# karenyang/GCN-VAE

Measured on NVIDIA B200. Metric: train edges/s (fwd+bwd) + eval triples/s, FB15k-237 shape, 1/2/4/8 B200, higher is better.
Workload: dtype f32

## Files before the change

### gcn-vae_b200/_lib.py

```python
import ctypes
import os

import torch

HERE = os.path.dirname(os.path.abspath(__file__))
LIB_PATH = os.path.join(HERE, "libkgvae_b200.so")

_P, _I, _F, _L, _Z = ctypes.c_void_p, ctypes.c_int, ctypes.c_float, ctypes.c_longlong, ctypes.c_size_t

_SIGNATURES = {
    "kg_last_error": (ctypes.c_char_p, []),
    "kg_version": (_I, []),
    "kg_device_info": (_I, [_P, _P, _P]),
    "kg_peer_alloc": (_I, [_Z, _P, _P]),
    "kg_peer_open": (_I, [_P, _P]),
    "kg_peer_close": (_I, [_P]),
    "kg_peer_free": (_I, [_P]),
    "kg_graph_build_workspace_bytes": (_Z, [_I]),
    "kg_graph_build": (_I, [_P, _P, _P, _I, _I, _I, _P, _P, _P, _P, _P, _P, _P, _P, _P, _P, _P, _Z, _P]),
    "kg_graph_index_workspace_bytes": (_Z, [_I]),
    "kg_graph_index": (_I, [_P, _P, _P, _P, _I, _I, _I, _P, _P, _P, _P, _P, _P, _P, _Z, _P]),
    "kg_embedding_fwd": (_I, [_P, _P, _I, _I, _P, _P]),
    "kg_embedding_bwd": (_I, [_P, _P, _I, _I, _P, _P]),
    "kg_bdd_weight_layouts": (_I, [_P, _I, _I, _I, _I, _P, _P, _P]),
    "kg_bdd_rel_fwd": (_I, [_P, _P, _I, _P, _I, _P, _P, _I, _I, _I, _P, _I, _P]),
    "kg_bdd_rel_bwd": (_I, [_P, _P, _I, _P, _P, _I, _P, _P, _I, _I, _I, _P, _P, _I, _P]),
    "kg_bdd_rel_fwd_cols": (_I, [_P, _P, _I, _P, _I, _I, _I, _I, _I, _P, _I, _P]),
    "kg_bdd_rel_bwd_cols": (_I, [_P, _P, _P, _I, _P, _I, _I, _I, _I, _I, _P, _P, _I, _P]),
    "kg_bdd_layouts_needed": (_I, [_I, _I, _I]),
    "kg_graph_rel_tiled_workspace_bytes": (_Z, [_I]),
    "kg_graph_rel_tiled": (_I, [_P, _P, _P, _P, _I, _I, _I, _I, _I, _P, _P, _Z, _P]),
    "kg_basis_id_fwd": (_I, [_P, _P, _P, _P, _P, _I, _I, _I, _I, _P, _P]),
    "kg_basis_id_bwd": (_I, [_P, _P, _P, _P, _P, _I, _I, _I, _I, _P, _P, _P]),
    "kg_basis_id_src_eligible": (_I, [_I, _I, _I]),
    "kg_basis_id_src_fwd": (_I, [_P, _P, _P, _P, _I, _I, _I, _I, _P, _P]),
    "kg_basis_id_src_bwd": (_I, [_P, _P, _P, _P, _P, _I, _I, _I, _I, _P, _P, _P]),
    "kg_basis_dense_fwd": (_I, [_P, _P, _I, _P, _I, _I, _I, _P, _P]),
    "kg_basis_dense_bwd": (_I, [_P, _P, _P, _I, _P, _I, _I, _I, _P, _P, _P]),
    "kg_act_dropout_bwd": (_I, [_P, _P, _P, _I, _L, _P, _P]),
    "kg_act_dropout_bwd_colsum": (_I, [_P, _P, _P, _I, _I, _I, _P, _P, _P, _Z, _P]),
    "kg_colsum_workspace_bytes": (_Z, [_I, _I]),
    "kg_colsum": (_I, [_P, _I, _I, _P, _P, _Z, _P]),
    "kg_gemm_f32_workspace_bytes": (_Z, [_I, _I, _I]),
    "kg_gemm_f32": (_I, [_P, _I, _I, _P, _I, _I, _P, _I, _I, _I, _I, _P, _P, _I, _P, _I, _P, _Z, _P]),
    "kg_gemm_f32_uses_tensor_cores": (_I, [_I, _I, _I]),
    "kg_gemm_prep_bytes": (_Z, [_I, _I]),
    "kg_gemm_prepare": (_I, [_P, _I, _I, _I, _P, _Z, _P]),
    "kg_gemm_f32_prepared_workspace_bytes": (_Z, [_I, _I, _I]),
    "kg_gemm_f32_prepared": (_I, [_P, _I, _P, _I, _P, _I, _I, _I, _I, _P, _P, _I, _P, _I, _P, _Z, _P]),
    "kg_reparam_fwd": (_I, [_P, _P, _I, _I, _P, _P, _P, _P]),
    "kg_reparam_bwd": (_I, [_P, _P, _P, _P, _P, _P, _I, _I, _P, _P]),
    "kg_kl_mog_fwd": (_I, [_P, _P, _P, _P, _I, _I, _I, _P, _P, _P, _P]),
    "kg_kl_mog_bwd": (_I, [_P, _P, _P, _P, _P, _P, _F, _I, _I, _I, _P, _P, _P, _P, _P]),
    "kg_kl_mog_bwd_fused": (_I, [_P, _P, _P, _P, _P, _P, _F, _I, _I, _I, _P, _P, _P, _P, _P, _P, _P]),
    "kg_iaf_update_fwd": (_I, [_P, _P, _P, _P, _I, _I, _P, _P, _P]),
    "kg_iaf_update_bwd": (_I, [_P, _P, _P, _P, _P, _I, _I, _P, _P, _P, _P]),
    "kg_reverse_columns": (_I, [_P, _I, _I, _P, _P]),
    "kg_distmult_score": (_I, [_P, _P, _P, _I, _I, _P, _P, _P]),
    "kg_reduce_workspace_bytes": (_Z, [_L]),
    "kg_bce_logits_fwd": (_I, [_P, _P, _I, _P, _P, _P, _Z, _P]),
    "kg_sum_squares": (_I, [_P, _L, _P, _P, _Z, _P]),
    "kg_sum": (_I, [_P, _L, _P, _P, _Z, _P]),
    "kg_triplet_index_workspace_bytes": (_Z, [_I]),
    "kg_triplet_index": (_I, [_P, _I, _I, _I, _P, _P, _P, _P, _Z, _P]),
    "kg_distmult_bce_workspace_bytes": (_Z, [_I]),
    "kg_distmult_bce_fwd": (_I, [_P, _P, _P, _P, _I, _I, _P, _P, _P, _P, _P, _P, _P, _P, _Z, _P]),
    "kg_distmult_bwd_dz": (_I, [_P, _P, _P, _P, _P, _I, _I, _P, _P]),
    "kg_triplet_index_trailing": (_I, [_P, _I, _I, _I, _P, _P, _P, _P, _Z, _P]),
    "kg_distmult_bce_fwd_lead": (_I, [_P, _P, _P, _P, _I, _I, _P, _P, _P, _P, _P, _P, _P, _P, _Z, _P]),
    "kg_distmult_bwd_dz_trailing": (_I, [_P, _P, _P, _P, _P, _I, _I, _P, _P]),
    "kg_distmult_bwd_dw": (_I, [_P, _P, _P, _I, _I, _P, _P]),
    "kg_distmult_rank_workspace_bytes": (_Z, [_I, _I, _I]),
    "kg_distmult_rank": (_I, [_P, _P, _P, _P, _P, _I, _I, _I, _P, _I, _I, _P, _P, _P, _Z, _P, _P, _P]),
    "kg_probe_l2": (_I, [_P, _P, _I, _I, _L, _I, _P, _P]),
    "kg_set_tc_terms": (_I, [_I]),
    "kg_distmult_topk_workspace_bytes": (_Z, [_I, _I, _I, _I]),
    "kg_distmult_topk": (_I, [_P, _P, _P, _P, _I, _I, _I, _P, _I, _P, _Z, _P, _P, _P]),
}

_lib = None


def lib():
    global _lib
    if _lib is None:
        if not os.path.exists(LIB_PATH):
            raise RuntimeError(
                f"kgvae_b200: {LIB_PATH} is missing - build it with "
                "`python -c 'import __graft_entry__ as g; g.build()'` (there is no CPU fallback)")
        handle = ctypes.CDLL(LIB_PATH)
        for name, (res, args) in _SIGNATURES.items():
            fn = getattr(handle, name)
            fn.restype, fn.argtypes = res, args
        _lib = handle
    return _lib


KERNELS_PER_CALL = {
    "kg_graph_build": 14, "kg_graph_index": 10, "kg_graph_rel_tiled": 5, "kg_triplet_index": 13, "kg_triplet_index_trailing": 18, "kg_distmult_bce_fwd": 5, "kg_distmult_bce_fwd_lead": 5, "kg_colsum": 2, "kg_act_dropout_bwd_colsum": 1,
    "kg_gemm_f32": 5,
    "kg_gemm_prepare": 2,
    "kg_kl_mog_fwd": 2, "kg_bce_logits_fwd": 2, "kg_sum_squares": 2, "kg_sum": 2, "kg_distmult_rank": 3, "kg_distmult_topk": 5,
}
launches = 0
profile = None


_seen_dev = None


def call(name, *args, tag=None):
    global launches, _seen_dev
    handle = lib()
    if _seen_dev is not None:
        dev, _seen_dev = _seen_dev, None
        if dev != torch.cuda.current_device():
            raise RuntimeError(f"kgvae_b200: {name} was given tensors on cuda:{dev} while the current device is "
                               f"cuda:{torch.cuda.current_device()} (use torch.cuda.set_device / torch.cuda.device)")
    if profile is not None:
        ev0, ev1 = torch.cuda.Event(enable_timing=True), torch.cuda.Event(enable_timing=True)
        ev0.record()
    rc = getattr(handle, name)(*args)
    if rc != 0:
        raise RuntimeError(f"{name} failed ({rc}): {handle.kg_last_error().decode()}")
    launches += KERNELS_PER_CALL.get(name, 1)
    if profile is not None:
        ev1.record()
        profile.setdefault(tag or name, []).append((ev0, ev1))


def ptr(t, dtype=None):
    if t is None:
        return None
    if not t.is_cuda:
        raise RuntimeError("kgvae_b200 ops need CUDA tensors (no CPU fallback)")
# ... 34 lines not shown
```

### gcn-vae_b200/csrc/latent.cu

```cuda
#include "common.cuh"

static constexpr int kThreads = 256;
static constexpr int kMaxMix = 16;
#define KG_LOG_SQRT_2PI 0.91893853320467274178f

__global__ void reparam_fwd_kernel(const float* __restrict__ h2, const float* __restrict__ eps, int n,
                                   int h, float* __restrict__ zm, float* __restrict__ zv,
                                   float* __restrict__ z) {
  long long t = (long long)blockIdx.x * blockDim.x + threadIdx.x;
  if (t >= (long long)n * h) return;
  int i = (int)(t / h), d = (int)(t % h);
  const float m = h2[(size_t)i * 2 * h + d];
  const float v = kg_softplus(h2[(size_t)i * 2 * h + h + d]) + 1e-8f;
  zm[t] = m;
  zv[t] = v;
  z[t] = m + eps[t] * sqrtf(v);
}

__global__ void reparam_bwd_kernel(const float* __restrict__ h2, const float* __restrict__ eps,
                                   const float* __restrict__ zv, const float* __restrict__ dz,
                                   const float* __restrict__ dmean, const float* __restrict__ dvar,
                                   int n, int h, float* __restrict__ dh2) {
  long long t = (long long)blockIdx.x * blockDim.x + threadIdx.x;
  if (t >= (long long)n * h) return;
  int i = (int)(t / h), d = (int)(t % h);
  const float g = dz ? dz[t] : 0.f;
  float gm = g, gv = g * eps[t] * 0.5f / sqrtf(zv[t]);
  if (dmean) gm += dmean[t];
  if (dvar) gv += dvar[t];
  dh2[(size_t)i * 2 * h + d] = gm;
  dh2[(size_t)i * 2 * h + h + d] = gv * kg_sigmoid(h2[(size_t)i * 2 * h + h + d]);
}
// ... 210 lines not shown
static void launch_kl_bwd(dim3 grid, cudaStream_t st, const float* z, const float* zm, const float* zv, const float* z_pre,
                          const float* ws, const float* resp, float scale, int n, int h, int k, const float* coefs,
                          const float* add, float* dz, float* dmean, float* dvar, float* dz_pre) {
  if (k <= 4) kl_mog_bwd_kernel<4><<<grid, 128, 0, st>>>(z, zm, zv, z_pre, ws, resp, scale, n, h, k, coefs, add, dz, dmean, dvar, dz_pre);
  else if (k <= 8) kl_mog_bwd_kernel<8><<<grid, 128, 0, st>>>(z, zm, zv, z_pre, ws, resp, scale, n, h, k, coefs, add, dz, dmean, dvar, dz_pre);
  else if (k <= 12) kl_mog_bwd_kernel<12><<<grid, 128, 0, st>>>(z, zm, zv, z_pre, ws, resp, scale, n, h, k, coefs, add, dz, dmean, dvar, dz_pre);
  else kl_mog_bwd_kernel<16><<<grid, 128, 0, st>>>(z, zm, zv, z_pre, ws, resp, scale, n, h, k, coefs, add, dz, dmean, dvar, dz_pre);
}

extern "C" int kg_kl_mog_bwd(const float* z, const float* z_mean, const float* z_var,
                             const float* z_pre, const float* prior_ws, const float* resp, float scale,
                             int n, int h, int k, float* dz, float* dmean, float* dvar, float* dz_pre,
                             void* stream) {
  KG_REQUIRE(n >= 0 && h > 0 && k > 0 && k <= kMaxMix, "kl bwd: need 0 < k <= 16");
  if (n == 0) return KG_OK;
  dim3 grid(kg_div_up(n, kKlRows), kg_div_up(h, 128));
  launch_kl_bwd(grid, kg_stream(stream), z, z_mean, z_var, z_pre, prior_ws, resp, scale, n, h, k, nullptr, nullptr, dz,
                dmean, dvar, dz_pre);
  KG_LAUNCH_OK();
  return KG_OK;
}

extern "C" int kg_kl_mog_bwd_fused(const float* z, const float* z_mean, const float* z_var,
                                   const float* z_pre, const float* prior_ws, const float* resp, float scale,
                                   int n, int h, int k, const float* coefs, const float* add, float* dz,
                                   float* dmean, float* dvar, float* dz_pre, void* stream) {
  KG_REQUIRE(n >= 0 && h > 0 && k > 0 && k <= kMaxMix, "kl bwd: need 0 < k <= 16");
  KG_REQUIRE(coefs != nullptr, "kl bwd fused: coefs is required");
  if (n == 0) return KG_OK;
  dim3 grid(kg_div_up(n, kKlRows), kg_div_up(h, 128));
  launch_kl_bwd(grid, kg_stream(stream), z, z_mean, z_var, z_pre, prior_ws, resp, scale, n, h, k, coefs, add, dz, dmean,
                dvar, dz_pre);
  KG_LAUNCH_OK();
  return KG_OK;
}

__global__ void __launch_bounds__(kThreads)
iaf_update_fwd_kernel(const float* __restrict__ z, const float* __restrict__ net,
                      const float* __restrict__ x_old, const int* __restrict__ col_mult, int n, int d,
                      float* __restrict__ x_new, float* __restrict__ log_det) {
  const int row = (int)(((long long)blockIdx.x * blockDim.x + threadIdx.x) >> 5);
  const int lane = threadIdx.x & 31;
  if (row >= n) return;
  const float* mu = net + (size_t)row * 2 * d;
  const float* alpha = mu + d;
  float s = 0.f;
  for (int j = lane; j < d; j += 32) {
    const float al = alpha[j];
    s += al;
    const size_t off = (size_t)row * d + j;
    if (__ldg(col_mult + j) == 0) x_new[off] = x_old[off];
    else x_new[off] = z[off] * expf(al + mu[j]);
  }
  if (log_det) {
    s = kg_warp_sum(s);
    if (lane == 0) log_det[row] = s;
  }
}

__global__ void iaf_update_bwd_kernel(const float* __restrict__ z, const float* __restrict__ net,
                                      const float* __restrict__ dx_new,
                                      const float* __restrict__ dlog_det,
                                      const int* __restrict__ col_mult, int n, int d,
                                      float* __restrict__ dz, float* __restrict__ dnet,
                                      float* __restrict__ dx_old) {
  long long t = (long long)blockIdx.x * blockDim.x + threadIdx.x;
// ... 58 lines not shown
```

### gcn-vae_b200/link_predict.py

```python
import argparse
import time

import numpy as np
import torch
import torch.nn as nn

from . import datasets, ops, utils
from .model import KGVAE, RGCN


class LinkPredict(nn.Module):
    def __init__(self, model_class, in_dim, h_dim, num_rels, num_bases=-1, num_hidden_layers=1,
                 dropout=0, use_cuda=True, reg_param=0, kl_param=0, mmd_param=0, k=1, n_flows=0):
        super().__init__()
        kwargs = dict(num_nodes=in_dim, h_dim=h_dim, out_dim=h_dim, num_rels=num_rels * 2,
                      num_bases=num_bases, num_hidden_layers=num_hidden_layers, dropout=dropout,
                      use_self_loop=use_cuda, use_cuda=use_cuda)
        if model_class is KGVAE:
            kwargs.update(k=k, n_flows=n_flows)
        self.encoder = model_class(**kwargs)
        self.reg_param, self.kl_param, self.mmd_param = reg_param, kl_param, mmd_param
        self.w_relation = nn.Parameter(torch.Tensor(num_rels, h_dim))
        self.use_cuda, self.k, self.n_flows = use_cuda, k, n_flows
        nn.init.xavier_uniform_(self.w_relation, gain=nn.init.calculate_gain("relu"))

    def grad_buckets(self, group=None, average=True, sharded=()):
        from . import parallel
        skip = {id(p) for p in sharded}
        enc = self.encoder
        named = dict(self.named_parameters())
        pick = lambda prefix: [p for n, p in named.items() if n.startswith(prefix) and p.requires_grad and id(p) not in skip]
        head = [p for n, p in named.items() if p.requires_grad and id(p) not in skip and
                not n.startswith(("encoder.rconv_layer_", "encoder.input_layer", "encoder.layers"))]
        order = [head, pick("encoder.rconv_layer_2"), pick("encoder.rconv_layer_1"), pick("encoder.layers"),
                 pick("encoder.input_layer")]
        params = [p for p in self.parameters() if p.requires_grad and id(p) not in skip]
        return parallel.GradBuckets(params, buckets=[b for b in order if b], group=group, average=average)

    def release_graph(self):
        enc = self.encoder
        for name in ("z_mean", "z_sigma", "log_det_sum", "flow_log_prob"):
            v = getattr(enc, name, None)
            if isinstance(v, torch.Tensor) and v.grad_fn is not None:
                setattr(enc, name, v.detach())

    def _flow_shift(self):
        if self.n_flows > 0 and isinstance(self.encoder, KGVAE):
            return self.encoder.get_flow_log_prob()
        return None

    def calc_score(self, embedding, triplets, shift=None):
        trip = ops.as_i32(triplets, embedding.device)
        return ops.DistMultScoreFn.apply(embedding, self.w_relation, trip, shift)

    def forward(self, g, h, r, norm):
        return self.encoder.forward(g, h, r, norm)

    def regularization_loss(self, embedding):
        return ops.MeanSquareFn.apply(embedding) + ops.MeanSquareFn.apply(self.w_relation)

    def get_loss(self, g, embed, triplets, labels):
        if getattr(g, "partition", None) is not None:
            return self._get_loss_partitioned(g.partition, embed, triplets, labels)
        trip = ops.as_i32(triplets, embed.device)
        lab = torch.as_tensor(labels, dtype=torch.float32, device=embed.device)
        zero = lambda: torch.zeros(1, device=embed.device)
        enc = self.encoder
        if isinstance(enc, KGVAE) and embed.requires_grad:
            flp = enc.flow_log_prob if enc.n_flows > 0 else None
            head, predict_loss, reg_loss, kl_core = ops.LossHeadFn.apply(
                embed, enc.z_mean, enc.z_sigma, enc.z_pre, self.w_relation, trip, lab, self._flow_shift(),
                self.reg_param, self.kl_param)
            kl = (kl_core if flp is None else kl_core + flp) if self.kl_param > 0 else zero()
            mmd = enc.get_mmd(embed) if self.mmd_param > 0 else zero()
            loss = head
            if self.kl_param > 0 and flp is not None:
                loss = loss + self.kl_param * flp
            if self.mmd_param > 0:
                loss = loss + self.mmd_param * mmd
            return loss, predict_loss, kl, mmd
        predict_loss = ops.DistMultBceFn.apply(embed, self.w_relation, trip, lab, self._flow_shift())
        reg_loss = self.regularization_loss(embed)
        kl = self.encoder.get_kl(embed) if self.kl_param > 0 else zero()
        mmd = self.encoder.get_mmd(embed) if self.mmd_param > 0 else zero()
        loss = predict_loss + self.reg_param * reg_loss + self.kl_param * kl + self.mmd_param * mmd
        return loss, predict_loss, kl, mmd


    def _get_loss_partitioned(self, part, embed, triplets, labels):
        from . import parallel
        dev = embed.device
        trip = ops.as_i32(triplets, dev)
        lab = torch.as_tensor(labels, dtype=torch.float32, device=dev)
        counts = torch.tensor([float(trip.shape[0])], device=dev)
        torch.distributed.all_reduce(counts, group=part.group)
        pending_z = parallel.allgather_rows_start(embed.detach(), part)
        frac = part.n_local / part.n_global
        reg_loss = ops.MeanSquareFn.apply(embed) * frac + ops.MeanSquareFn.apply(self.w_relation) / part.world_size
        zero = lambda: torch.zeros(1, device=dev)
        if self.kl_param > 0:
# ... 286 lines not shown
```

### gcn-vae_b200/model.py

```python
import random

import numpy as np
import torch
import torch.nn as nn
import torch.nn.functional as F

from . import ops, utils
from .flow_network import MADE, PermuteLayer
from .nn import RelGraphConv


class EmbeddingLayer(nn.Module):

    def __init__(self, num_nodes, h_dim):
        super().__init__()
        self.embedding = nn.Embedding(num_nodes, h_dim)

    def forward(self, g, h, r, norm):
        ids = ops.as_i32(h.reshape(-1), self.embedding.weight.device)
        return ops.EmbeddingFn.apply(self.embedding.weight, ids)


class KGVAE(nn.Module):

    def __init__(self, num_nodes, h_dim, out_dim, num_rels, num_bases, num_hidden_layers=1,
                 dropout=0, use_self_loop=False, use_cuda=True, k=10, n_flows=0):
        super().__init__()
        self.num_nodes, self.h_dim, self.out_dim, self.num_rels = num_nodes, h_dim, out_dim, num_rels
        self.num_bases = None if num_bases < 0 else num_bases
        self.num_hidden_layers = num_hidden_layers
        self.dropout = dropout
        self.use_self_loop, self.use_cuda = use_self_loop, use_cuda
        self.k = k
        self.flow_log_prob = None
        self.preset_eps = None
        self.build_encoder()
        self.z_pre = nn.Parameter(torch.randn(1, 2 * k, h_dim) / np.sqrt(k * h_dim))
        self.pi = nn.Parameter(torch.ones(k) / k, requires_grad=False)
        self.n_flows = n_flows
        if n_flows > 0:
            self.build_iaf()

    def build_iaf(self):
        blocks = []
        for _ in range(self.n_flows):
            blocks += [MADE(self.h_dim, self.h_dim, self.n_flows), PermuteLayer(self.h_dim)]
        self.nf = nn.Sequential(*blocks)

    def build_encoder(self):
        self.input_layer = EmbeddingLayer(self.num_nodes, self.h_dim)
        self.rconv_layer_1 = RelGraphConv(self.h_dim, self.h_dim, self.num_rels, "bdd",
                                          self.num_bases, activation=nn.ReLU(), self_loop=True,
                                          dropout=self.dropout)
        self.rconv_layer_2 = RelGraphConv(self.h_dim, self.h_dim * 2, self.num_rels, "bdd",
                                          self.num_bases, activation=nn.Identity(), self_loop=True,
                                          dropout=self.dropout)

    def forward(self, g, h, r, norm):
        self.node_id = h.squeeze()
        x = self.input_layer(g, h, r, norm)
        x = self.rconv_layer_1(g, x, r, norm)
        x = self.rconv_layer_2(g, x, r, norm)
        eps = self.preset_eps
        if eps is None:
            part = getattr(g, "partition", None)
            gen = None if part is None else part.noise_generator(x.device)
            eps = torch.randn((x.shape[0], self.h_dim), device=x.device, generator=gen)
        self.z_mean, self.z_sigma, z = ops.ReparamFn.apply(x, eps)
        if self.n_flows > 0:
            log_det_sum = None
            for flow in self.nf:
                z, log_det = flow.forward(z)
                if isinstance(flow, MADE):
                    log_det_sum = log_det if log_det_sum is None else log_det_sum + log_det
            self.log_det_sum = log_det_sum
            part = getattr(g, "partition", None)
            if part is None:
                self.flow_log_prob = torch.mean(log_det_sum)
            else:
                from . import parallel
                self.flow_log_prob = parallel.AllReduceSumFn.apply(log_det_sum.sum(), part.group) / part.n_global
        return z

    def get_kl(self, z):
        kl = ops.KlMogFn.apply(z, self.z_mean, self.z_sigma, self.z_pre)
        return kl if self.flow_log_prob is None else kl + self.flow_log_prob

    def get_flow_log_prob(self):
        return self.flow_log_prob

    def compute_kernel(self, x, y):
        d = x.size(1)
        diff = x.unsqueeze(1) - y.unsqueeze(0)
        return torch.exp(-diff.pow(2).mean(2) / float(d))

    def get_mmd(self, z):
        m_mix, s_mix = utils.gaussian_parameters(self.z_pre, dim=1)
        num_sample = 200
        z_pri = utils.sample_gaussian(m_mix, s_mix, repeat=num_sample // self.k)
        if self.n_flows > 0:
# ... 91 lines not shown
```

### gcn-vae_b200/ops.py

```python
import os

import torch

from . import _lib as L


def _c(t):
    return t if t.is_contiguous() else t.contiguous()


class tensor_core_terms:

    def __init__(self, terms):
        self.terms = int(terms)

    def __enter__(self):
        self.old = L.lib().kg_set_tc_terms(self.terms)
        return self

    def __exit__(self, *exc):
        L.lib().kg_set_tc_terms(self.old)
        return False


# ... 353 lines not shown
        if ctx.has_bias and ctx.needs_input_grad[3]:
            dbias = dbias_fused
        if isinstance(pending, list):
            dx = torch.cat([p_.wait() for p_ in pending], dim=1) if pending else None
        elif pending is not None:
            dx = pending.wait()
        return dx, dw, dloop, dbias, None, None, None, None, None, None, None


class ReparamFn(torch.autograd.Function):

    @staticmethod
    def forward(ctx, h2, eps):
        h2, eps = _c(h2), _c(eps)
        n, h = eps.shape
        zm, zv, z = (torch.empty_like(eps) for _ in range(3))
        L.call("kg_reparam_fwd", L.f32(h2), L.f32(eps), n, h, L.f32(zm), L.f32(zv), L.f32(z), L.stream())
        ctx.save_for_backward(h2, eps, zv)
        return zm, zv, z

    @staticmethod
    def backward(ctx, gm, gv, gz):
        h2, eps, zv = ctx.saved_tensors
        n, h = eps.shape
        gm = None if gm is None else _c(gm)
        gv = None if gv is None else _c(gv)
        gz = None if gz is None else _c(gz)
        dh2 = torch.empty_like(h2)
        L.call("kg_reparam_bwd", L.f32(h2), L.f32(eps), L.f32(zv), L.f32(gz), L.f32(gm), L.f32(gv),
               n, h, L.f32(dh2), L.stream())
        return dh2, None


class KlMogFn(torch.autograd.Function):

    @staticmethod
    def forward(ctx, z, z_mean, z_var, z_pre):
        z, z_mean, z_var = _c(z), _c(z_mean), _c(z_var)
        zp = _c(z_pre.reshape(-1, z_pre.shape[-1]))
        n, h = z.shape
        k = zp.shape[0] // 2
        dev = z.device
        ws = torch.empty((3, k, h), dtype=torch.float32, device=dev)
        rows = torch.empty(n, dtype=torch.float32, device=dev)
        resp = torch.empty((n, k), dtype=torch.float32, device=dev)
        L.call("kg_kl_mog_fwd", L.f32(z), L.f32(z_mean), L.f32(z_var), L.f32(zp), n, h, k, L.f32(ws),
               L.f32(rows), L.f32(resp), L.stream())
        ctx.save_for_backward(z, z_mean, z_var, zp, ws, resp)
        ctx.pre_shape = z_pre.shape
        return _reduce("kg_sum", rows) / n

    @staticmethod
    def backward(ctx, g):
        z, z_mean, z_var, zp, ws, resp = ctx.saved_tensors
        n, h = z.shape
        k = zp.shape[0] // 2
        dz, dm, dv = (torch.empty_like(z) for _ in range(3))
        dzp = torch.zeros_like(zp)
        L.call("kg_kl_mog_bwd", L.f32(z), L.f32(z_mean), L.f32(z_var), L.f32(zp), L.f32(ws),
               L.f32(resp), 1.0 / n, n, h, k, L.f32(dz), L.f32(dm), L.f32(dv), L.f32(dzp), L.stream())
        return dz * g, dm * g, dv * g, (dzp * g).view(ctx.pre_shape)


class LinearFn(torch.autograd.Function):

    @staticmethod
# ... 228 lines not shown
        ctx.shift_shape = None if shift is None else shift.shape
        ctx.pre_shape = None if z_pre is None else z_pre.shape
        return loss, pred, reg, kl

    @staticmethod
    def backward(ctx, g_loss, g_pred, g_reg, g_kl):
        saved = ctx.saved_tensors
        z, w, dz_pred, dw, out = saved[:5]
        n, h = z.shape
        zero = torch.zeros((), dtype=torch.float32, device=z.device)
        g_loss, g_pred, g_reg, g_kl = ((zero if t is None else t.reshape(()).to(torch.float32))
                                       for t in (g_loss, g_pred, g_reg, g_kl))
        c_pred = g_loss + g_pred
        c_reg = g_loss * ctx.reg_param + g_reg
        c_kl = g_loss * ctx.kl_param + g_kl
        dm = dv = dzp = None
        if ctx.use_kl:
            z_mean, z_var, zp, pws, resp = saved[5:]
            k = zp.shape[0] // 2
            coefs = torch.stack([c_kl, c_pred, c_reg * (2.0 / z.numel())]).contiguous()
            dz, dm, dv = (torch.empty_like(z) for _ in range(3))
            dzp = torch.zeros_like(zp)
            L.call("kg_kl_mog_bwd_fused", L.f32(z), L.f32(z_mean), L.f32(z_var), L.f32(zp), L.f32(pws), L.f32(resp),
                   1.0 / n, n, h, k, L.f32(coefs), L.f32(dz_pred), L.f32(dz), L.f32(dm), L.f32(dv), L.f32(dzp),
                   L.stream(), tag="kg_kl_mog_bwd")
            dzp = dzp.view(ctx.pre_shape)
        else:
            dz = torch.addcmul(dz_pred * c_pred, z, c_reg * (2.0 / z.numel()))
        dwo = torch.addcmul(dw * c_pred, w, c_reg * (2.0 / w.numel()))
        dshift = (out[1] * c_pred).reshape(ctx.shift_shape) if ctx.shift_shape is not None else None
        return dz, dm, dv, dzp, dwo, None, None, dshift, None, None


class BceLogitsFn(torch.autograd.Function):

    @staticmethod
    def forward(ctx, score, labels):
        score, labels = _c(score), _c(labels)
        n = score.numel()
        loss = torch.empty((), dtype=torch.float32, device=score.device)
        dscore = torch.empty_like(score)
        ws = L.workspace(L.lib().kg_reduce_workspace_bytes(n), score.device)
        L.call("kg_bce_logits_fwd", L.f32(score), L.f32(labels), n, L.f32(loss), L.f32(dscore),
               L.ptr(ws), ws.numel(), L.stream())
        ctx.save_for_backward(dscore)
        return loss

    @staticmethod
    def backward(ctx, g):
        (dscore,) = ctx.saved_tensors
        return dscore * g, None


class MeanSquareFn(torch.autograd.Function):

    @staticmethod
    def forward(ctx, x):
        x = _c(x)
        ctx.save_for_backward(x)
        return _reduce("kg_sum_squares", x) / x.numel()

    @staticmethod
    def backward(ctx, g):
        (x,) = ctx.saved_tensors
        return x * (g * (2.0 / x.numel()))

# ... 27 lines not shown
```

### include/kgvae_b200.h

```cpp
#ifndef KGVAE_B200_H_
#define KGVAE_B200_H_

#include <stddef.h>
#include <stdint.h>

#ifdef __cplusplus
extern "C" {
#endif

#define KG_OK 0
#define KG_ERR_INVALID -1
#define KG_ERR_CUDA -2
#define KG_ERR_WORKSPACE -3

const char* kg_last_error(void);
int kg_version(void);
int kg_device_info(int* sm_count, int* cc_major, int* cc_minor);
int kg_peer_alloc(size_t bytes, void** ptr, unsigned char* handle_out );
int kg_peer_open(const unsigned char* handle , void** ptr);
int kg_peer_close(void* ptr);
int kg_peer_free(void* ptr);

size_t kg_graph_build_workspace_bytes(int n_triplets);
int kg_graph_build(const int32_t* src, const int32_t* rel, const int32_t* dst, int n_triplets,
// ... 68 lines not shown
int kg_colsum(const float* x, int rows, int cols, float* out, void* workspace, size_t workspace_bytes,
              void* stream);

size_t kg_gemm_f32_workspace_bytes(int M, int N, int K);
int kg_gemm_f32(const float* A, int lda, int trans_a, const float* B, int ldb, int trans_b,
                float* C, int ldc, int M, int N, int K,
                const float* bias, const float* addend, int relu, const float* mask,
                int accumulate, void* workspace, size_t workspace_bytes, void* stream);

int kg_gemm_f32_uses_tensor_cores(int M, int N, int K);
size_t kg_gemm_prep_bytes(int rows, int cols);
int kg_gemm_prepare(const float* src, int ld, int rows, int cols, void* prep, size_t prep_bytes, void* stream);
size_t kg_gemm_f32_prepared_workspace_bytes(int M, int N, int K);
int kg_gemm_f32_prepared(const void* prep_a, int trans_a, const void* prep_b, int trans_b,
                         float* C, int ldc, int M, int N, int K,
                         const float* bias, const float* addend, int relu, const float* mask,
                         int accumulate, void* workspace, size_t workspace_bytes, void* stream);

int kg_reparam_fwd(const float* h2, const float* eps, int n, int h, float* z_mean, float* z_var,
                   float* z, void* stream);
int kg_reparam_bwd(const float* h2, const float* eps, const float* z_var, const float* dz,
                   const float* dmean, const float* dvar, int n, int h, float* dh2, void* stream);

int kg_kl_mog_fwd(const float* z, const float* z_mean, const float* z_var, const float* z_pre,
                  int n, int h, int k, float* prior_ws, float* kl_rows, float* resp, void* stream);
int kg_kl_mog_bwd(const float* z, const float* z_mean, const float* z_var, const float* z_pre,
                  const float* prior_ws, const float* resp, float scale, int n, int h, int k,
                  float* dz, float* dmean, float* dvar, float* dz_pre, void* stream);
int kg_kl_mog_bwd_fused(const float* z, const float* z_mean, const float* z_var, const float* z_pre,
                        const float* prior_ws, const float* resp, float scale, int n, int h, int k,
                        const float* coefs, const float* add, float* dz, float* dmean, float* dvar,
                        float* dz_pre, void* stream);

int kg_iaf_update_fwd(const float* z, const float* net_out, const float* x_old,
                      const int32_t* col_mult, int n, int d, float* x_new, float* log_det,
                      void* stream);
int kg_iaf_update_bwd(const float* z, const float* net_out, const float* dx_new,
                      const float* dlog_det , const int32_t* col_mult, int n, int d,
                      float* dz, float* dnet_out, float* dx_old, void* stream);
int kg_reverse_columns(const float* x, int n, int d, float* out, void* stream);

int kg_distmult_score(const float* z, const float* w, const int32_t* triplets, int n_triplets, int h,
                      const float* shift , float* score, void* stream);
size_t kg_reduce_workspace_bytes(long long n);
int kg_bce_logits_fwd(const float* score, const float* labels, int n, float* loss_out, float* dscore,
                      void* workspace, size_t workspace_bytes, void* stream);
int kg_sum_squares(const float* x, long long n, float* out, void* workspace, size_t workspace_bytes,
                   void* stream);
int kg_sum(const float* x, long long n, float* out, void* workspace, size_t workspace_bytes,
           void* stream);
size_t kg_triplet_index_workspace_bytes(int n_triplets);
int kg_triplet_index(const int32_t* triplets, int n_triplets, int n_nodes, int n_rels,
                     void* rs_rec, int32_t* ent_ptr, void* ent_pack,
                     void* workspace, size_t workspace_bytes, void* stream);
size_t kg_distmult_bce_workspace_bytes(int n_triplets);
int kg_distmult_bce_fwd(const float* z, const float* w, const void* rs_rec, const float* labels,
                        int n_triplets, int h, const float* shift ,
                        float* score_out, float* g_out, float* dw, float* dz, float* loss_out,
                        float* gsum_out, void* workspace, size_t workspace_bytes, void* stream);
int kg_distmult_bwd_dz(const float* z, const float* w, const float* gscore, const int32_t* ent_ptr,
                       const void* ent_pack, int n_nodes, int h, float* dz, void* stream);

int kg_triplet_index_trailing(const int32_t* triplets, int n_triplets, int n_nodes, int n_rels,
                              void* rs_rec, int32_t* trail_ptr, void* trail_pack,
                              void* workspace, size_t workspace_bytes, void* stream);
int kg_distmult_bce_fwd_lead(const float* z, const float* w, const void* rs_rec, const float* labels,
// ... 32 lines not shown
```

Measured before the change: 66.44 million.

## Fuse reparameterization, MoG KL and z-norm into single latent fwd/bwd kernels

Adds a fused latent forward kernel that computes the reparameterized z, the variance, the mixture-of-Gaussians KL with responsibilities, and the sum of squares of z in one pass, using a last-block ticket reduction. A fused backward recomputes z from h2 and eps and produces dh2 plus per-chunk prior gradients, which a small kernel then reduces. A new loss-head autograd path uses these when there are no flows and no partition. This removes several separate kernel launches and extra round trips through memory for the reparam, KL and regularizer terms, at the cost of more code paths and a new gradient routing to check for correctness.

```diff
diff --git a/gcn-vae_b200/_lib.py b/gcn-vae_b200/_lib.py
--- a/gcn-vae_b200/_lib.py
+++ b/gcn-vae_b200/_lib.py
@@ -53,6 +53,9 @@
     "kg_kl_mog_fwd": (_I, [_P, _P, _P, _P, _I, _I, _I, _P, _P, _P, _P]),
     "kg_kl_mog_bwd": (_I, [_P, _P, _P, _P, _P, _P, _F, _I, _I, _I, _P, _P, _P, _P, _P]),
     "kg_kl_mog_bwd_fused": (_I, [_P, _P, _P, _P, _P, _P, _F, _I, _I, _I, _P, _P, _P, _P, _P, _P, _P]),
+    "kg_latent_workspace_bytes": (_Z, [_I, _I]),
+    "kg_latent_fwd": (_I, [_P, _P, _P, _I, _I, _I, _P, _P, _P, _P, _P, _Z, _P]),
+    "kg_latent_bwd": (_I, [_P, _P, _P, _P, _P, _P, _I, _I, _I, _P, _P, _P, _Z, _P]),
     "kg_iaf_update_fwd": (_I, [_P, _P, _P, _P, _I, _I, _P, _P, _P]),
     "kg_iaf_update_bwd": (_I, [_P, _P, _P, _P, _P, _I, _I, _P, _P, _P, _P]),
     "kg_reverse_columns": (_I, [_P, _I, _I, _P, _P]),
@@ -100,7 +103,7 @@
     "kg_graph_build": 14, "kg_graph_index": 10, "kg_graph_rel_tiled": 5, "kg_triplet_index": 13, "kg_triplet_index_trailing": 18, "kg_distmult_bce_fwd": 5, "kg_distmult_bce_fwd_lead": 5, "kg_colsum": 2, "kg_act_dropout_bwd_colsum": 1,
     "kg_gemm_f32": 5,
     "kg_gemm_prepare": 2,
-    "kg_kl_mog_fwd": 2, "kg_bce_logits_fwd": 2, "kg_sum_squares": 2, "kg_sum": 2, "kg_distmult_rank": 3, "kg_distmult_topk": 5,
+    "kg_kl_mog_fwd": 2, "kg_latent_fwd": 2, "kg_latent_bwd": 2, "kg_bce_logits_fwd": 2, "kg_sum_squares": 2, "kg_sum": 2, "kg_distmult_rank": 3, "kg_distmult_topk": 5,
 }
 launches = 0
 profile = None
diff --git a/gcn-vae_b200/csrc/latent.cu b/gcn-vae_b200/csrc/latent.cu
--- a/gcn-vae_b200/csrc/latent.cu
+++ b/gcn-vae_b200/csrc/latent.cu
@@ -1,3 +1,5 @@
+#include <algorithm>
+
 #include "common.cuh"
 
 static constexpr int kThreads = 256;
@@ -274,6 +276,300 @@
   launch_kl_bwd(grid, kg_stream(stream), z, z_mean, z_var, z_pre, prior_ws, resp, scale, n, h, k, coefs, add, dz, dmean,
                 dvar, dz_pre);
   KG_LAUNCH_OK();
+  return KG_OK;
+}
+
+static constexpr int kLatFwdThreads = 128;
+static constexpr int kLatWarpRows = 2;
+static constexpr int kLatFwdMaxCtas = 2048;
+static constexpr int kLatBwdChunks = 296;
+static constexpr int kLatBwdCols = 128;
+
+static size_t lat_prior_floats(int k, int h) { return (size_t)3 * k * h + k; }
+static size_t lat_fwd_part_offset(int k, int h) { return kg_align_up(lat_prior_floats(k, h), 64); }
+static size_t lat_bwd_part_offset(int k, int h) { return lat_fwd_part_offset(k, h) + 2 * kLatFwdMaxCtas; }
+
+extern "C" size_t kg_latent_workspace_bytes(int k, int h) {
+  if (k <= 0 || h <= 0) return 0;
+  return sizeof(float) * (lat_bwd_part_offset(k, h) + (size_t)kLatBwdChunks * 2 * k * h);
+}
+
+__global__ void latent_prior_kernel(const float* __restrict__ z_pre, int k, int h, float* __restrict__ ws) {
+  const int i = threadIdx.x >> 5, lane = threadIdx.x & 31;
+  if (i >= k) return;
+  float* inv2v = ws + (size_t)k * h;
+  float* lsq = ws + (size_t)2 * k * h;
+  float lsum = 0.f;
+  for (int d = lane * 4; d < h; d += 128) {
+    float l[4];
+#pragma unroll
+    for (int c = 0; c < 4; ++c) {
+      const size_t t = (size_t)i * h + d + c;
+      const float v = kg_softplus(z_pre[(size_t)k * h + t]) + 1e-8f;
+      ws[t] = v;
+      inv2v[t] = 1.f / (2.f * v);
+      l[c] = lsq[t] = logf(sqrtf(v));
+    }
+    lsum += (l[0] + l[1]) + (l[2] + l[3]);
+  }
+  lsum = kg_warp_sum(lsum);
+  if (lane == 0) ws[(size_t)3 * k * h + i] = lsum + (float)h * KG_LOG_SQRT_2PI;
+}
+
+template <int KM>
+__global__ void __launch_bounds__(kLatFwdThreads, 3)
+latent_fwd_kernel(const float* __restrict__ h2, const float* __restrict__ eps, const float* __restrict__ z_pre,
+                  const float* __restrict__ ws, int n, int h, int k, float* __restrict__ z, float* __restrict__ zv,
+                  float* __restrict__ resp, float* __restrict__ part, unsigned int* __restrict__ ticket,
+                  float* __restrict__ out) {
+  const int lane = threadIdx.x & 31, warp = threadIdx.x >> 5;
+  const float* inv2v = ws + (size_t)k * h;
+  const float* cst = ws + (size_t)3 * k * h;
+  float kl_acc = 0.f, zsq = 0.f;
+  const long long groups = ((long long)n + kLatWarpRows - 1) / kLatWarpRows;
+  for (long long grp = (long long)blockIdx.x * (kLatFwdThreads / 32) + warp; grp < groups;
+       grp += (long long)gridDim.x * (kLatFwdThreads / 32)) {
+    const long long row0 = grp * kLatWarpRows;
+    float a[kLatWarpRows], b[kLatWarpRows][KM];
+#pragma unroll
+    for (int q = 0; q < kLatWarpRows; ++q) {
+      a[q] = 0.f;
+#pragma unroll
+      for (int i = 0; i < KM; ++i) b[q][i] = 0.f;
+    }
+#pragma unroll 1
+    for (int d = lane * 4; d < h; d += 128) {
+      float zc[kLatWarpRows][4];
+#pragma unroll
+      for (int q = 0; q < kLatWarpRows; ++q) {
+        const long long row = min(row0 + q, (long long)n - 1);
+        const float4 m4 = *reinterpret_cast<const float4*>(h2 + (size_t)row * 2 * h + d);
+        const float4 s4 = *reinterpret_cast<const float4*>(h2 + (size_t)row * 2 * h + h + d);
+        const float4 e4 = *reinterpret_cast<const float4*>(eps + (size_t)row * h + d);
+        const float mc[4] = {m4.x, m4.y, m4.z, m4.w}, sc[4] = {s4.x, s4.y, s4.z, s4.w}, ec[4] = {e4.x, e4.y, e4.z, e4.w};
+        float vc[4];
+#pragma unroll
+        for (int c = 0; c < 4; ++c) {
+          const float m = mc[c];
+          const float v = kg_softplus(sc[c]) + 1e-8f;
+          vc[c] = v;
+          zc[q][c] = m + ec[c] * sqrtf(v);
+          const float t = zc[q][c] - m;
+          a[q] += -__fdividef(t * t, 2.f * v) - 0.5f * __logf(v) - KG_LOG_SQRT_2PI;
+        }
+        if (row0 + q < n) {
+          const size_t off = (size_t)row * h + d;
+          *reinterpret_cast<float4*>(z + off) = make_float4(zc[q][0], zc[q][1], zc[q][2], zc[q][3]);
+          if (zv) *reinterpret_cast<float4*>(zv + off) = make_float4(vc[0], vc[1], vc[2], vc[3]);
+#pragma unroll
+          for (int c = 0; c < 4; ++c) zsq = fmaf(zc[q][c], zc[q][c], zsq);
+        }
+      }
+#pragma unroll
+      for (int i = 0; i < KM; ++i)
+        if (i < k) {
+          const size_t po = (size_t)i * h + d;
+          const float4 t0 = __ldg(reinterpret_cast<const float4*>(z_pre + po)),
+                       t1 = __ldg(reinterpret_cast<const float4*>(inv2v + po));
+          const float pm[4] = {t0.x, t0.y, t0.z, t0.w}, iv[4] = {t1.x, t1.y, t1.z, t1.w};
+#pragma unroll
+          for (int q = 0; q < kLatWarpRows; ++q)
+#pragma unroll
+            for (int c = 0; c < 4; ++c) {
+              const float u = zc[q][c] - pm[c];
+              b[q][i] = fmaf(-(u * u), iv[c], b[q][i]);
+            }
+        }
+    }
+#pragma unroll
+    for (int q = 0; q < kLatWarpRows; ++q) {
+      const long long row = row0 + q;
+      const float aq = kg_warp_sum(a[q]);
+      float mx = -INFINITY;
+#pragma unroll
+      for (int i = 0; i < KM; ++i)
+        if (i < k) {
+          b[q][i] = kg_warp_sum(b[q][i]) - __ldg(cst + i);
+          mx = fmaxf(mx, b[q][i]);
+        }
+      float se = 0.f;
+#pragma unroll
+      for (int i = 0; i < KM; ++i)
+        if (i < k) se += expf(b[q][i] - mx);
+      const float lse = mx + logf(se);
+      if (row < n) {
+        kl_acc += aq - (lse - logf((float)k));
+#pragma unroll
+        for (int i = 0; i < KM; ++i)
+          if (i < k && lane == (i & 31)) resp[(size_t)row * k + i] = expf(b[q][i] - lse);
+      }
+    }
+  }
+  __shared__ float red[2][kLatFwdThreads / 32];
+  __shared__ bool last;
+  zsq = kg_warp_sum(zsq);
+  if (lane == 0) { red[0][warp] = kl_acc; red[1][warp] = zsq; }
+  __syncthreads();
+  if (threadIdx.x == 0) {
+    float s0 = 0.f, s1 = 0.f;
+#pragma unroll
+    for (int w = 0; w < kLatFwdThreads / 32; ++w) { s0 += red[0][w]; s1 += red[1][w]; }
+    part[blockIdx.x] = s0;
+    part[kLatFwdMaxCtas + blockIdx.x] = s1;
+    __threadfence();
+    last = atomicAdd(ticket, 1u) == gridDim.x - 1;
+  }
+  __syncthreads();
+  if (!last || warp != 0) return;
+  __threadfence();
+  float s0 = 0.f, s1 = 0.f;
+  for (int c = lane; c < gridDim.x; c += 32) {
+    s0 += __ldcg(part + c);
+    s1 += __ldcg(part + kLatFwdMaxCtas + c);
+  }
+  s0 = kg_warp_sum(s0);
+  s1 = kg_warp_sum(s1);
+  if (lane == 0) {
+    out[0] = s0 / (float)n;
+    out[1] = s1 / ((float)n * (float)h);
+  }
+}
+
+extern "C" int kg_latent_fwd(const float* h2, const float* eps, const float* z_pre, int n, int h, int k, float* z,
+                             float* z_var, float* resp, float* out, void* workspace, size_t workspace_bytes,
+                             void* stream) {
+  KG_REQUIRE(n > 0 && h > 0 && k > 0 && k <= kMaxMix, "latent fwd: need n > 0, h > 0, 0 < k <= 16");
+  KG_REQUIRE(h % 4 == 0 && ((reinterpret_cast<uintptr_t>(h2) | reinterpret_cast<uintptr_t>(eps) |
+                             reinterpret_cast<uintptr_t>(z_pre) | reinterpret_cast<uintptr_t>(z) |
+                             reinterpret_cast<uintptr_t>(z_var) | reinterpret_cast<uintptr_t>(workspace)) & 15) == 0,
+             "latent fwd: needs h % 4 == 0 and 16-byte aligned rows");
+  KG_REQUIRE(workspace_bytes >= kg_latent_workspace_bytes(k, h), "latent fwd: workspace too small");
+  cudaStream_t st = kg_stream(stream);
+  float* ws = reinterpret_cast<float*>(workspace);
+  float* part = ws + lat_fwd_part_offset(k, h);
+  unsigned int* ticket = reinterpret_cast<unsigned int*>(ws + lat_bwd_part_offset(k, h));
+  KG_CUDA(cudaMemsetAsync(ticket, 0, sizeof(unsigned int), st));
+  latent_prior_kernel<<<1, 32 * k, 0, st>>>(z_pre, k, h, ws);
+  KG_LAUNCH_OK();
+  const long long groups = ((long long)n + kLatWarpRows - 1) / kLatWarpRows;
+  const int grid = (int)std::min<long long>((groups + kLatFwdThreads / 32 - 1) / (kLatFwdThreads / 32), kLatFwdMaxCtas);
+#define KG_LAT_FWD(KM_) \
+  latent_fwd_kernel<KM_><<<grid, kLatFwdThreads, 0, st>>>(h2, eps, z_pre, ws, n, h, k, z, z_var, resp, part, ticket, out)
+  if (k <= 4) KG_LAT_FWD(4);
+  else if (k <= 8) KG_LAT_FWD(8);
+  else if (k <= 12) KG_LAT_FWD(12);
+  else KG_LAT_FWD(16);
+#undef KG_LAT_FWD
+  KG_LAUNCH_OK();
+  return KG_OK;
+}
+
+static constexpr int kLatBwdRowTile = 32;
+
+template <int KM>
+__global__ void __launch_bounds__(kLatBwdCols)
+latent_bwd_kernel(const float* __restrict__ h2, const float* __restrict__ eps, const float* __restrict__ z_pre,
+                  const float* __restrict__ ws, const float* __restrict__ resp, const float* __restrict__ dz_pred,
+                  const float* __restrict__ coefs, int n, int h, int k, int rows_per_chunk, float* __restrict__ dh2,
+                  float* __restrict__ part) {
+  __shared__ float rs[kLatBwdRowTile * KM];
+  const int d = blockIdx.y * kLatBwdCols + threadIdx.x;
+  const bool col = d < h;
+  const float scale = __ldg(coefs) / (float)n, c_pred = __ldg(coefs + 1), c_z = __ldg(coefs + 2);
+  float pm[KM], ipv[KM], gpm[KM], acc[KM];
+#pragma unroll
+  for (int i = 0; i < KM; ++i) {
+    pm[i] = i < k && col ? z_pre[(size_t)i * h + d] : 0.f;
+    ipv[i] = i < k && col ? 1.f / ws[(size_t)i * h + d] : 0.f;
+    gpm[i] = 0.f;
+    acc[i] = 0.f;
+  }
+  const long long r0 = (long long)blockIdx.x * rows_per_chunk, r1 = min((long long)n, r0 + rows_per_chunk);
+  for (long long t0 = r0; t0 < r1; t0 += kLatBwdRowTile) {
+    const int nr = (int)min((long long)kLatBwdRowTile, r1 - t0);
+    __syncthreads();
+    for (int j = threadIdx.x; j < nr * k; j += kLatBwdCols) rs[(j / k) * KM + j % k] = __ldg(resp + t0 * k + j);
+    __syncthreads();
+    if (!col) continue;
+#pragma unroll 4
+    for (int q = 0; q < nr; ++q) {
+      const size_t row = (size_t)(t0 + q);
+      const float m = h2[row * 2 * h + d], s = h2[row * 2 * h + h + d], e = eps[row * h + d];
+      const float add = dz_pred[row * h + d];
+      const float v = kg_softplus(s) + 1e-8f;
+      const float sq = sqrtf(v);
+      const float zc = m + e * sq;
+      const float t = zc - m;
+      const float iv = __frcp_rn(v);
+      const float tiv = t * iv;
+      float gmix = 0.f;
+#pragma unroll
+      for (int i = 0; i < KM; ++i)
+        if (i < k) {
+          const float ri = rs[q * KM + i];
+          const float u = zc - pm[i];
+          const float qq = ri * (u * ipv[i]);
+          gmix += qq;
+          gpm[i] -= qq;
+          acc[i] += fmaf(qq, u, -ri);
+        }
+      const float rest = c_z * zc + c_pred * add;
+      const float gz = scale * (gmix - tiv) + rest;
+      dh2[row * 2 * h + d] = scale * gmix + rest;
+      const float gv = gz * e * 0.5f / sq + scale * 0.5f * iv * (t * tiv - 1.f);
+      dh2[row * 2 * h + h + d] = gv * kg_sigmoid(s);
+    }
+  }
+  if (!col) return;
+  float* p = part + (size_t)blockIdx.x * 2 * k * h;
+#pragma unroll
+  for (int i = 0; i < KM; ++i)
+    if (i < k) {
+      p[(size_t)i * h + d] = gpm[i];
+      p[(size_t)(k + i) * h + d] = acc[i];
+    }
+}
+
+__global__ void latent_prior_bwd_kernel(const float* __restrict__ z_pre, const float* __restrict__ ws,
+                                        const float* __restrict__ part, int chunks, const float* __restrict__ coefs,
+                                        int n, int h, int k, float* __restrict__ dz_pre) {
+  const int t = blockIdx.x * blockDim.x + threadIdx.x;
+  if (t >= 2 * k * h) return;
+  float s = 0.f;
+  for (int c = 0; c < chunks; ++c) s += part[(size_t)c * 2 * k * h + t];
+  const float scale = __ldg(coefs) / (float)n;
+  if (t < k * h) {
+    dz_pre[t] = scale * s;
+  } else {
+    const int j = t - k * h;
+    dz_pre[t] = scale * (-0.5f * (1.f / ws[j]) * s) * kg_sigmoid(z_pre[t]);
+  }
+}
+
+extern "C" int kg_latent_bwd(const float* h2, const float* eps, const float* z_pre, const float* resp,
+                             const float* dz_pred, const float* coefs, int n, int h, int k, float* dh2, float* dz_pre,
+                             void* workspace, size_t workspace_bytes, void* stream) {
+  KG_REQUIRE(n > 0 && h > 0 && k > 0 && k <= kMaxMix, "latent bwd: need n > 0, h > 0, 0 < k <= 16");
+  KG_REQUIRE(coefs != nullptr && dz_pred != nullptr, "latent bwd: coefs and dz_pred are required");
+  KG_REQUIRE(workspace_bytes >= kg_latent_workspace_bytes(k, h), "latent bwd: workspace too small");
+  cudaStream_t st = kg_stream(stream);
+  float* ws = reinterpret_cast<float*>(workspace);
+  float* part = ws + lat_bwd_part_offset(k, h);
+  const int rows_per_chunk = kg_div_up(n, kLatBwdChunks);
+  const dim3 grid(kg_div_up(n, rows_per_chunk), kg_div_up(h, kLatBwdCols));
+#define KG_LAT_BWD(KM_) \
+  latent_bwd_kernel<KM_><<<grid, kLatBwdCols, 0, st>>>(h2, eps, z_pre, ws, resp, dz_pred, coefs, n, h, k, rows_per_chunk, dh2, part)
+  if (k <= 4) KG_LAT_BWD(4);
+  else if (k <= 8) KG_LAT_BWD(8);
+  else if (k <= 12) KG_LAT_BWD(12);
+  else KG_LAT_BWD(16);
+#undef KG_LAT_BWD
+  KG_LAUNCH_OK();
+  if (dz_pre) {
+    latent_prior_bwd_kernel<<<kg_div_up(2LL * k * h, kThreads), kThreads, 0, st>>>(z_pre, ws, part, (int)grid.x, coefs,
+                                                                                   n, h, k, dz_pre);
+    KG_LAUNCH_OK();
+  }
   return KG_OK;
 }
 
diff --git a/gcn-vae_b200/link_predict.py b/gcn-vae_b200/link_predict.py
--- a/gcn-vae_b200/link_predict.py
+++ b/gcn-vae_b200/link_predict.py
@@ -43,6 +43,8 @@
             v = getattr(enc, name, None)
             if isinstance(v, torch.Tensor) and v.grad_fn is not None:
                 setattr(enc, name, v.detach())
+        if getattr(enc, "latent", None) is not None:
+            enc.latent = None
 
     def _flow_shift(self):
         if self.n_flows > 0 and isinstance(self.encoder, KGVAE):
@@ -66,6 +68,14 @@
         lab = torch.as_tensor(labels, dtype=torch.float32, device=embed.device)
         zero = lambda: torch.zeros(1, device=embed.device)
         enc = self.encoder
+        lat = getattr(enc, "latent", None) if isinstance(enc, KGVAE) else None
+        if lat is not None and lat.z is embed and embed.requires_grad:
+            head, predict_loss, reg_loss, kl_core = ops.FusedLossHeadFn.apply(
+                embed, lat.h2, lat.eps, enc.z_pre, self.w_relation, trip, lab, None, self.reg_param, self.kl_param, lat)
+            kl = kl_core if self.kl_param > 0 else zero()
+            mmd = enc.get_mmd(embed) if self.mmd_param > 0 else zero()
+            loss = head + self.mmd_param * mmd if self.mmd_param > 0 else head
+            return loss, predict_loss, kl, mmd
         if isinstance(enc, KGVAE) and embed.requires_grad:
             flp = enc.flow_log_prob if enc.n_flows > 0 else None
             head, predict_loss, reg_loss, kl_core = ops.LossHeadFn.apply(
diff --git a/gcn-vae_b200/model.py b/gcn-vae_b200/model.py
--- a/gcn-vae_b200/model.py
+++ b/gcn-vae_b200/model.py
@@ -34,6 +34,7 @@
         self.k = k
         self.flow_log_prob = None
         self.preset_eps = None
+        self.latent = None
         self.build_encoder()
         self.z_pre = nn.Parameter(torch.randn(1, 2 * k, h_dim) / np.sqrt(k * h_dim))
         self.pi = nn.Parameter(torch.ones(k) / k, requires_grad=False)
@@ -66,6 +67,14 @@
             part = getattr(g, "partition", None)
             gen = None if part is None else part.noise_generator(x.device)
             eps = torch.randn((x.shape[0], self.h_dim), device=x.device, generator=gen)
+        self.latent = None
+        if (self.n_flows == 0 and getattr(g, "partition", None) is None and self.training and torch.is_grad_enabled()
+                and x.requires_grad and ops.latent_fusable(x, eps)):
+            self.latent = ops.LatentState()
+            self.z_sigma, z = ops.LatentFn.apply(x, eps, self.z_pre, self.latent)
+            self.z_mean = x[:, :self.h_dim]
+            self.latent.z, self.latent.h2, self.latent.eps = z, x, eps
+            return z
         self.z_mean, self.z_sigma, z = ops.ReparamFn.apply(x, eps)
         if self.n_flows > 0:
             log_det_sum = None
diff --git a/gcn-vae_b200/ops.py b/gcn-vae_b200/ops.py
--- a/gcn-vae_b200/ops.py
+++ b/gcn-vae_b200/ops.py
@@ -409,6 +409,48 @@
         return dh2, None
 
 
+def latent_fusable(h2, eps):
+    h = eps.shape[1]
+    return (h % 4 == 0 and h2.is_contiguous() and eps.is_contiguous() and h2.shape[0] > 0
+            and h2.data_ptr() % 16 == 0 and eps.data_ptr() % 16 == 0)
+
+
+class LatentState:
+    z = h2 = eps = resp = out = ws = None
+
+
+class LatentFn(torch.autograd.Function):
+
+    @staticmethod
+    def forward(ctx, h2, eps, z_pre, state):
+        n, h = eps.shape
+        zp = _c(z_pre.reshape(-1, h))
+        k = zp.shape[0] // 2
+        dev = h2.device
+        zv, z = torch.empty_like(eps), torch.empty_like(eps)
+        state.resp = torch.empty((n, k), dtype=torch.float32, device=dev)
+        state.out = torch.empty(2, dtype=torch.float32, device=dev)
+        state.ws = L.workspace(L.lib().kg_latent_workspace_bytes(k, h), dev)
+        L.call("kg_latent_fwd", L.f32(h2), L.f32(eps), L.f32(zp), n, h, k, L.f32(z), L.f32(zv), L.f32(state.resp),
+               L.f32(state.out), L.ptr(state.ws), state.ws.numel(), L.stream())
+        ctx.set_materialize_grads(False)
+        ctx.save_for_backward(h2, eps, zv)
+        return zv, z
+
+    @staticmethod
+    def backward(ctx, gv, gz):
+        if gv is None and gz is None:
+            return None, None, None, None
+        h2, eps, zv = ctx.saved_tensors
+        n, h = eps.shape
+        gv = None if gv is None else _c(gv)
+        gz = None if gz is None else _c(gz)
+        dh2 = torch.empty_like(h2)
+        L.call("kg_reparam_bwd", L.f32(h2), L.f32(eps), L.f32(zv), L.f32(gz), None, L.f32(gv), n, h, L.f32(dh2),
+               L.stream())
+        return dh2, None, None, None
+
+
 class KlMogFn(torch.autograd.Function):
 
     @staticmethod
@@ -703,6 +745,50 @@
         return dz, dm, dv, dzp, dwo, None, None, dshift, None, None
 
 
+class FusedLossHeadFn(torch.autograd.Function):
+
+    @staticmethod
+    def forward(ctx, z, h2, eps, z_pre, w, triplets, labels, shift, reg_param, kl_param, state):
+        w, labels = _c(w), _c(labels)
+        n, h = z.shape
+        out, dw, dz_pred = distmult_bce_pass(z, w, triplets, labels, shift, True)
+        pred = out[0].clone()
+        reg = state.out[1] + _reduce("kg_sum_squares", w) / w.numel()
+        use_kl = kl_param > 0
+        if use_kl:
+            kl = state.out[0].clone()
+            loss = pred + reg_param * reg + kl_param * kl
+        else:
+            kl = torch.zeros((), dtype=torch.float32, device=z.device)
+            loss = pred + reg_param * reg
+        ctx.save_for_backward(h2, eps, _c(z_pre.reshape(-1, h)), w, dz_pred, dw, out, state.resp, state.ws)
+        ctx.use_kl, ctx.reg_param, ctx.kl_param = use_kl, float(reg_param), float(kl_param)
+        ctx.shift_shape = None if shift is None else shift.shape
+        ctx.pre_shape = z_pre.shape
+        return loss, pred, reg, kl
+
+    @staticmethod
+    def backward(ctx, g_loss, g_pred, g_reg, g_kl):
+        h2, eps, zp, w, dz_pred, dw, out, resp, ws = ctx.saved_tensors
+        n, h = eps.shape
+        k = zp.shape[0] // 2
+        zero = torch.zeros((), dtype=torch.float32, device=h2.device)
+        g_loss, g_pred, g_reg, g_kl = ((zero if t is None else t.reshape(()).to(torch.float32))
+                                       for t in (g_loss, g_pred, g_reg, g_kl))
+        c_pred = g_loss + g_pred
+        c_reg = g_loss * ctx.reg_param + g_reg
+        c_kl = g_loss * ctx.kl_param + g_kl if ctx.use_kl else zero
+        coefs = torch.stack([c_kl, c_pred, c_reg * (2.0 / (n * h))]).contiguous()
+        dh2 = torch.empty_like(h2)
+        dzp = torch.empty_like(zp) if ctx.use_kl else None
+        L.call("kg_latent_bwd", L.f32(h2), L.f32(eps), L.f32(zp), L.f32(resp), L.f32(dz_pred), L.f32(coefs), n, h, k,
+               L.f32(dh2), L.f32(dzp), L.ptr(ws), ws.numel(), L.stream(), tag="kg_latent_bwd")
+        dwo = torch.addcmul(dw * c_pred, w, c_reg * (2.0 / w.numel()))
+        dshift = (out[1] * c_pred).reshape(ctx.shift_shape) if ctx.shift_shape is not None else None
+        dzp = None if dzp is None else dzp.view(ctx.pre_shape)
+        return None, dh2, None, dzp, dwo, None, None, dshift, None, None, None
+
+
 class BceLogitsFn(torch.autograd.Function):
 
     @staticmethod
diff --git a/include/kgvae_b200.h b/include/kgvae_b200.h
--- a/include/kgvae_b200.h
+++ b/include/kgvae_b200.h
@@ -124,6 +124,13 @@
                         const float* coefs, const float* add, float* dz, float* dmean, float* dvar,
                         float* dz_pre, void* stream);
 
+size_t kg_latent_workspace_bytes(int k, int h);
+int kg_latent_fwd(const float* h2, const float* eps, const float* z_pre, int n, int h, int k, float* z,
+                  float* z_var, float* resp, float* out, void* workspace, size_t workspace_bytes, void* stream);
+int kg_latent_bwd(const float* h2, const float* eps, const float* z_pre, const float* resp, const float* dz_pred,
+                  const float* coefs, int n, int h, int k, float* dh2, float* dz_pre, void* workspace,
+                  size_t workspace_bytes, void* stream);
+
 int kg_iaf_update_fwd(const float* z, const float* net_out, const float* x_old,
                       const int32_t* col_mult, int n, int d, float* x_new, float* log_det,
                       void* stream);
```

After: 67.16 million, median of 6. 1.01x the previous value.
